# NVIDIA/OpenSeq2Seq

Hardware: AMD Instinct MI355X
Metric: audio-frames/sec/node Jasper10x5 bf16 (train step, objects = input feature frames) (higher is better)
Workload: dtype bf16; 1 GPU; Jasper 10x5 DR (jasper10x5_LibriSpeech_nvgrad_masks) full train step: log-mel front end from int16 PCM resident in HBM+fwd+bwd+NovoGrad/LARC/Backoff, B=32/GPU, durations U[2,16.7]s padded to the batch max, F=64, V=29; global_batch=32, parallelism=dp1, skipped_steps=0

## Files before the change

### openseq2seq_amd/csrc/conv1d_common.hpp

```cpp
#pragma once
#include <type_traits>

#include "os2s_common.hpp"

namespace os2s {

struct ConvArgs {
  const bf16_t* x;
  const bf16_t* w;
  void* y;
  const int32_t* in_len;
  const int32_t* out_len;
  const float* bias;
  float* stats;
  int B, Tin, Tout, Cin, Cout, K, stride, dil, padL;
  long long x_sb, x_st, y_sb, y_st;
  int out_f32, accumulate;
  int mtiles_per_b, MT, MT8, NT, nchunks, R, Rpad;
  int act;
  float keep_prob;
  unsigned long long seed;
  const bf16_t* residual;
  const bf16_t* mask_ref;
  float mask_scale;
  const bf16_t* stat_ref;
  float* ws_slabs;
  int* ws_cnt;
  int ws_nslabs, ncu;
  int force_split;
  unsigned long long* dbg;
  int dbg_fixed_w;
  int pp_tile = 0, pp_ok2 = 0, pp_ok3 = 0;
  float pp_c256 = 1.19f, pp_c2 = 0.90f, pp_c3 = 1.06f;
  int pp_prio = 0;
  float pp_dgrad_pen = 1.f;
  int tile_order = 0;
};

__device__ __forceinline__ void dma16(const void* gsrc, char* lds_wave_base) {
  __builtin_amdgcn_global_load_lds(
      (const __attribute__((address_space(1))) void*)gsrc,
      (__attribute__((address_space(3))) void*)lds_wave_base, 16, 0, 0);
}

constexpr size_t kEpiSplitBytes = 140 * 1024;
template <int BM, int BN, int NWIN, int NTHR>
constexpr size_t conv_epilogue_lds_bytes() {
  constexpr size_t OP = BN * 2 + 16;
  constexpr int EW = (NWIN * BM * OP > kEpiSplitBytes) ? 1 : NWIN;
  constexpr int RG = (NTHR / (BN / 2)) > 0 ? (NTHR / (BN / 2)) : 1;
  return (size_t)EW * BM * OP + (size_t)EW * RG * BN * 2 * 4;
}

constexpr int kMaxConvGroups = 16;
struct ConvGroup {
  const bf16_t* x;
  const bf16_t* w;
  void* y;
  float* stats;
  int Cin, Cout, accumulate, tile_begin;
  int x_st = 0, y_st = 0;
};
struct ConvGroupTable {
  int ngroups, total_tiles;
  ConvGroup g[kMaxConvGroups];
};
int launch_conv1x1_pp(hipStream_t stream, ConvArgs a, ConvGroupTable gt);

template <int BM, int BN, int WM, int WN, int NWIN>
__device__ __forceinline__ void conv_epilogue(const ConvArgs& p,
                                              f32x16 (&acc)[(BN / WN) / 32][((BM * NWIN) / WM) / 32],
                                              char* smem, int tid, int lane, int wid,
                                              const int (&wmid)[NWIN], int n0,
                                              const int (&wb)[NWIN], const int (&wt0)[NWIN]) {
  constexpr int NW = WM * WN, NTHR = NW * 64;
  constexpr int WTM = (BM * NWIN) / WM, WTN = BN / WN, MI = WTM / 32, NI = WTN / 32;
  const int wm = wid / WN, wn = wid % WN;
  constexpr bool STRADDLE = (BM % WTM) != 0;
  static_assert(!STRADDLE || (size_t)NWIN * BM * (BN * 2 + 16) <= kEpiSplitBytes,
                "a straddling wave layout needs all windows staged in one pass");
  const int my_win = (wm * WTM) / BM;
  const int row_in_win = (wm * WTM) % BM;
  const int my_b = (NWIN == 1 || my_win == 0) ? wb[0] : wb[NWIN - 1];
  const int my_t0 = (NWIN == 1 || my_win == 0) ? wt0[0] : wt0[NWIN - 1];
  const int my_mid = (NWIN == 1 || my_win == 0) ? wmid[0] : wmid[NWIN - 1];
  const int l31 = lane & 31, lhi = lane >> 5;
  if (p.out_f32) {
    const int b = my_b, t0 = my_t0;
    const int valid_rows = (my_mid >= 0) ? min(BM, p.Tout - t0) : 0;
    float* const yb = reinterpret_cast<float*>(p.y) + (long long)b * p.y_sb;
#pragma unroll
    for (int in = 0; in < NI; ++in)
#pragma unroll
      for (int im = 0; im < MI; ++im) {
        const int tt = row_in_win + im * 32 + l31;
#pragma unroll
        for (int e = 0; e < 16; ++e) {
          const int cc = n0 + wn * WTN + in * 32 + 8 * (e >> 2) + 4 * lhi + (e & 3);
          if (tt < valid_rows && cc < p.Cout) {
            float v = acc[in][im][e];
            if (p.bias) v += p.bias[cc];
            float* dst = yb + (long long)(t0 + tt) * p.y_st + cc;
            if (p.accumulate) v += *dst;
            *dst = v;
          }
        }
      }
    return;
  }

#ifdef OS2S_EPI_STAMPS
  unsigned long long* const est = (p.dbg && blockIdx.x < 2048) ? p.dbg + (size_t)blockIdx.x * 24 + 8 : nullptr;
  int esi = 0;
#define OS2S_EPI_STAMP() do { if (est && tid == 0 && esi < 16) est[esi] = __builtin_readcyclecounter(); ++esi; } while (0)
#else
#define OS2S_EPI_STAMP() do {} while (0)
#endif
  constexpr int OP = BN * 2 + 16;
  constexpr bool EPI_SPLIT = (size_t)NWIN * BM * OP > kEpiSplitBytes;
  constexpr int EW = EPI_SPLIT ? 1 : NWIN;
  char* const ot = smem;
#pragma unroll
  for (int w0 = 0; w0 < NWIN; w0 += EW) {
  OS2S_EPI_STAMP();
  __syncthreads();
  OS2S_EPI_STAMP();
  auto stage_tile = [&](auto DROP) {
  unsigned long long seed = p.seed;
  if constexpr (decltype(DROP)::value) asm volatile("" : "+s"(seed));
#pragma unroll
  for (int in = 0; in < NI; ++in)
#pragma unroll
    for (int im = 0; im < MI; ++im) {
      const int tt = wm * WTM + im * 32 + l31 - w0 * BM;
      const int b = my_b, t0 = my_t0 - (my_win - w0) * BM;
#pragma unroll
      for (int g = 0; g < 4; ++g) {
        const int cc = wn * WTN + in * 32 + 8 * g + 4 * lhi;
        float v0 = acc[in][im][4 * g + 0], v1 = acc[in][im][4 * g + 1];
        float v2 = acc[in][im][4 * g + 2], v3 = acc[in][im][4 * g + 3];
        if (p.bias) {
          const int gc = n0 + cc;
          if (gc + 3 < p.Cout) {
            v0 += p.bias[gc]; v1 += p.bias[gc + 1]; v2 += p.bias[gc + 2]; v3 += p.bias[gc + 3];
          }
        }
        if (p.act == 1) {
          v0 = fmaxf(v0, 0.f); v1 = fmaxf(v1, 0.f); v2 = fmaxf(v2, 0.f); v3 = fmaxf(v3, 0.f);
        } else if (p.act == 3) {
          v0 = fminf(fmaxf(v0, 0.f), 20.f); v1 = fminf(fmaxf(v1, 0.f), 20.f);
          v2 = fminf(fmaxf(v2, 0.f), 20.f); v3 = fminf(fmaxf(v3, 0.f), 20.f);
        }
        if constexpr (decltype(DROP)::value) {
          const long long e0 = ((long long)b * p.Tout + t0 + tt) * p.Cout + n0 + cc;
          const uint32_t bits = dropout_bits8(seed, (unsigned long long)(e0 >> 3), p.keep_prob) >>
                                (uint32_t)(e0 & 7);
          const float ik = 1.f / p.keep_prob;
          v0 = (bits & 1u) ? v0 * ik : 0.f;
          v1 = (bits & 2u) ? v1 * ik : 0.f;
          v2 = (bits & 4u) ? v2 * ik : 0.f;
          v3 = (bits & 8u) ? v3 * ik : 0.f;
        }
        u32x2 pk;
        pk[0] = pack2bf(v0, v1);
        pk[1] = pack2bf(v2, v3);
        *reinterpret_cast<u32x2*>(ot + tt * OP + cc * 2) = pk;
      }
    }
  };
  if constexpr (STRADDLE) {
    stage_tile(std::false_type{});
  } else if (my_win >= w0 && my_win < w0 + EW) {
    if (__builtin_amdgcn_readfirstlane(p.keep_prob < 1.f ? 1 : 0)) stage_tile(std::true_type{});
    else stage_tile(std::false_type{});
  }
  OS2S_EPI_STAMP();
  __syncthreads();
  OS2S_EPI_STAMP();

#pragma unroll
  for (int w = w0; w < w0 + EW; ++w) {
  const int b = wb[w], t0 = wt0[w];
  const int valid_rows = (wmid[w] >= 0) ? min(BM, p.Tout - t0) : 0;
  const char* const otw = ot + (w - w0) * BM * OP;
  bf16_t* const yb = reinterpret_cast<bf16_t*>(p.y) + (long long)b * p.y_sb;
  constexpr int NQ = (BM * (BN / 8) + NTHR - 1) / NTHR;
  static_assert((BM * (BN / 8)) % NTHR == 0, "whole number of chunks per thread");
  const bool inside = __builtin_amdgcn_readfirstlane((valid_rows == BM && n0 + BN <= p.Cout) ? 1 : 0);
  u32x4 v[NQ], ro[NQ], ao[NQ];
  if (inside) {
#pragma unroll
    for (int i = 0; i < NQ; ++i) {
      const int q = tid + i * NTHR;
      const int row = q / (BN / 8), c8 = q - row * (BN / 8);
      v[i] = *reinterpret_cast<const u32x4*>(otw + row * OP + c8 * 16);
      const long long off = (long long)(t0 + row) * p.y_st + n0 + c8 * 8;
      if (p.residual) ro[i] = *reinterpret_cast<const u32x4*>(p.residual + (long long)b * p.y_sb + off);
      if (p.accumulate) ao[i] = *reinterpret_cast<const u32x4*>(yb + off);
      if (p.mask_ref) ro[i] = *reinterpret_cast<const u32x4*>(p.mask_ref + (long long)b * p.y_sb + off);
    }
#pragma unroll
    for (int i = 0; i < NQ; ++i) {
      const int q = tid + i * NTHR;
      const int row = q / (BN / 8), c8 = q - row * (BN / 8);
      if (p.residual && !p.mask_ref) {
#pragma unroll
        for (int e = 0; e < 4; ++e)
          v[i][e] = pack2bf(bflo(v[i][e]) + bflo(ro[i][e]), bfhi(v[i][e]) + bfhi(ro[i][e]));
      }
      if (p.accumulate) {
#pragma unroll
        for (int e = 0; e < 4; ++e)
          v[i][e] = pack2bf(bflo(v[i][e]) + bflo(ao[i][e]), bfhi(v[i][e]) + bfhi(ao[i][e]));
      }
      if (p.mask_ref) {
#pragma unroll
        for (int e = 0; e < 4; ++e)
          v[i][e] = pack2bf(bflo(ro[i][e]) > 0.f ? bflo(v[i][e]) * p.mask_scale : 0.f,
                            bfhi(ro[i][e]) > 0.f ? bfhi(v[i][e]) * p.mask_scale : 0.f);
        if (p.stats) *reinterpret_cast<u32x4*>(const_cast<char*>(otw) + row * OP + c8 * 16) = v[i];
      }
      *reinterpret_cast<u32x4*>(yb + (long long)(t0 + row) * p.y_st + n0 + c8 * 8) = v[i];
    }
  } else {
    for (int i = 0; i < NQ; ++i) {
      const int q = tid + i * NTHR;
      const int row = q / (BN / 8), c8 = q - row * (BN / 8);
      const int gc = n0 + c8 * 8;
      if (row < valid_rows && gc < p.Cout) {
        u32x4 x = *reinterpret_cast<const u32x4*>(otw + row * OP + c8 * 16);
        bf16_t* dst = yb + (long long)(t0 + row) * p.y_st + gc;
        if (p.residual && !p.mask_ref) {
          const u32x4 o = *reinterpret_cast<const u32x4*>(
              p.residual + (long long)b * p.y_sb + (long long)(t0 + row) * p.y_st + gc);
#pragma unroll
          for (int e = 0; e < 4; ++e) x[e] = pack2bf(bflo(x[e]) + bflo(o[e]), bfhi(x[e]) + bfhi(o[e]));
        }
        if (p.accumulate) {
          const u32x4 o = *reinterpret_cast<const u32x4*>(dst);
#pragma unroll
          for (int e = 0; e < 4; ++e) x[e] = pack2bf(bflo(x[e]) + bflo(o[e]), bfhi(x[e]) + bfhi(o[e]));
        }
        if (p.mask_ref) {
          const u32x4 o = *reinterpret_cast<const u32x4*>(
              p.mask_ref + (long long)b * p.y_sb + (long long)(t0 + row) * p.y_st + gc);
#pragma unroll
          for (int e = 0; e < 4; ++e)
            x[e] = pack2bf(bflo(o[e]) > 0.f ? bflo(x[e]) * p.mask_scale : 0.f,
                           bfhi(o[e]) > 0.f ? bfhi(x[e]) * p.mask_scale : 0.f);
          if (p.stats) *reinterpret_cast<u32x4*>(const_cast<char*>(otw) + row * OP + c8 * 16) = x;
        }
        *reinterpret_cast<u32x4*>(dst) = x;
      }
    }
  }
  }

  OS2S_EPI_STAMP();
  if (p.stats && p.mask_ref) __syncthreads();
  if (p.stats) {
    constexpr int CP = BN / 2;
    constexpr int RG = (NTHR / CP) > 0 ? (NTHR / CP) : 1;
    constexpr int RPT = (BM + RG - 1) / RG;
    const int cp = tid % CP, rg = tid / CP;
#pragma unroll
    for (int w = w0; w < w0 + EW; ++w) {
      if (wmid[w] < 0) continue;
      const int valid_rows = min(BM, p.Tout - wt0[w]);
      const char* const otw = ot + (w - w0) * BM * OP;
      float s0 = 0.f, s1 = 0.f, q0 = 0.f, q1 = 0.f;
      if (rg < RG) {
        uint32_t vv[RPT];
#pragma unroll
        for (int i = 0; i < RPT; ++i) {
          const int row = rg + i * RG;
          vv[i] = row < valid_rows ? *reinterpret_cast<const uint32_t*>(otw + row * OP + cp * 4) : 0u;
        }
        if (p.stat_ref) {
          const bool cok = n0 + cp * 2 < p.Cout;
          const bf16_t* const rp = p.stat_ref + (long long)wb[w] * p.y_sb + (long long)wt0[w] * p.y_st + n0 + cp * 2;
          uint32_t rr[RPT];
#pragma unroll
          for (int i = 0; i < RPT; ++i) {
            const int row = rg + i * RG;
            rr[i] = (cok && row < valid_rows) ? *reinterpret_cast<const uint32_t*>(rp + (long long)row * p.y_st) : 0u;
          }
#pragma unroll
          for (int i = 0; i < RPT; ++i) {
            const float a = bflo(vv[i]), bb = bfhi(vv[i]);
            s0 += a; q0 += a * bflo(rr[i]);
            s1 += bb; q1 += bb * bfhi(rr[i]);
          }
        } else {
#pragma unroll
          for (int i = 0; i < RPT; ++i) {
            const float a = bflo(vv[i]), bb = bfhi(vv[i]);
            s0 += a; q0 += a * a;
            s1 += bb; q1 += bb * bb;
          }
        }
        float* sc = reinterpret_cast<float*>(smem + EW * BM * OP) + (size_t)(w - w0) * RG * BN * 2;
        sc[(rg * BN + cp * 2 + 0) * 2 + 0] = s0;
        sc[(rg * BN + cp * 2 + 0) * 2 + 1] = q0;
        sc[(rg * BN + cp * 2 + 1) * 2 + 0] = s1;
        sc[(rg * BN + cp * 2 + 1) * 2 + 1] = q1;
      }
    }
    OS2S_EPI_STAMP();
    __syncthreads();
    OS2S_EPI_STAMP();
#pragma unroll
    for (int w = w0; w < w0 + EW; ++w) {
      if (wmid[w] < 0) continue;
      const float* sc = reinterpret_cast<const float*>(smem + EW * BM * OP) + (size_t)(w - w0) * RG * BN * 2;
      for (int c = tid; c < BN; c += NTHR) {
        float s = 0.f, qq = 0.f;
#pragma unroll
        for (int g = 0; g < RG; ++g) {
          s += sc[(g * BN + c) * 2 + 0];
          qq += sc[(g * BN + c) * 2 + 1];
        }
        const int gc = n0 + c;
        if (gc < p.Cout) {
          p.stats[((long long)wmid[w] * 2 + 0) * p.Cout + gc] = s;
          p.stats[((long long)wmid[w] * 2 + 1) * p.Cout + gc] = qq;
        }
      }
    }
  }
  }
}

}
```

Baseline: 967,800 frames/sec.

## Fuse stats reduction into conv epilogue store pass with buffer loads and prefetch

Rewrites the conv epilogue's write-out phase so the per-channel sum/sumsq statistics are computed in the same pass that applies residual/accumulate/mask and stores the output. The separate stats pass that reread the staged tile from LDS, and the barrier before it, go away. Global reads and writes now use raw buffer loads and stores with range-clamped resources, which replaces the explicit boundary branches. The next batch's residual/accumulate/mask loads are issued before the current batch is stored, to overlap memory latency. When stats are enabled it switches to 8-byte pieces and processes two windows per half-block. This risks higher register pressure and subtle correctness issues in the reduction layout and out-of-range handling.

```diff
diff --git a/openseq2seq_amd/csrc/conv1d_common.hpp b/openseq2seq_amd/csrc/conv1d_common.hpp
--- a/openseq2seq_amd/csrc/conv1d_common.hpp
+++ b/openseq2seq_amd/csrc/conv1d_common.hpp
@@ -67,6 +67,14 @@
 };
 int launch_conv1x1_pp(hipStream_t stream, ConvArgs a, ConvGroupTable gt);
 
+__device__ __forceinline__ __amdgpu_buffer_rsrc_t epi_rsrc(const void* base, long long elem_off, int bytes) {
+  const unsigned long long a = (unsigned long long)base + (unsigned long long)elem_off * 2ull;
+  const unsigned lo = __builtin_amdgcn_readfirstlane((unsigned)a);
+  const unsigned hi = __builtin_amdgcn_readfirstlane((unsigned)(a >> 32));
+  return __builtin_amdgcn_make_buffer_rsrc((void*)(((unsigned long long)hi << 32) | lo), 0,
+                                           __builtin_amdgcn_readfirstlane(bytes), 0x00020000);
+}
+
 template <int BM, int BN, int WM, int WN, int NWIN>
 __device__ __forceinline__ void conv_epilogue(const ConvArgs& p,
                                               f32x16 (&acc)[(BN / WN) / 32][((BM * NWIN) / WM) / 32],
@@ -119,7 +127,10 @@
   constexpr int OP = BN * 2 + 16;
   constexpr bool EPI_SPLIT = (size_t)NWIN * BM * OP > kEpiSplitBytes;
   constexpr int EW = EPI_SPLIT ? 1 : NWIN;
+  constexpr int CP = BN / 2;
+  constexpr int RG = (NTHR / CP) > 0 ? (NTHR / CP) : 1;
   char* const ot = smem;
+
 #pragma unroll
   for (int w0 = 0; w0 < NWIN; w0 += EW) {
   OS2S_EPI_STAMP();
@@ -174,138 +185,163 @@
     if (__builtin_amdgcn_readfirstlane(p.keep_prob < 1.f ? 1 : 0)) stage_tile(std::true_type{});
     else stage_tile(std::false_type{});
   }
+  auto run_windows = [&](auto W16) {
+  constexpr bool WIDE = decltype(W16)::value;
+  constexpr int PB = WIDE ? 16 : 8, PD = PB / 4;
+  using piece_t = std::conditional_t<WIDE, u32x4, u32x2>;
+  constexpr int LR = BN * 2 / PB;
+  constexpr int TPW = WIDE ? NTHR : NTHR / 2;
+  constexpr int RGM = TPW / LR;
+  constexpr int RPT = BM / RGM;
+  static_assert(BM % RGM == 0 && TPW % 64 == 0 && (WIDE || RGM == RG), "whole waves per window; the chains of the sums");
+  constexpr int NROUND = WIDE ? EW : (EW + 1) / 2;
+  constexpr int NQB = WIDE ? ((NW > 4 || RPT % 2) ? RPT : RPT / 2) : ((NW > 4 && RPT % 16 == 0) ? 16 : 8);
+  static_assert(RPT % NQB == 0, "whole batches per window");
+  constexpr int NBT = RPT / NQB;
+  const int half = WIDE ? 0 : __builtin_amdgcn_readfirstlane(tid / TPW);
+  const int th = tid - half * TPW, c4 = th % LR, rg = th / LR;
+  const int y_st2 = (int)p.y_st * 2;
+  const int voff0 = (n0 + c4 * (PB / 2) < p.Cout) ? rg * y_st2 + (n0 + c4 * (PB / 2)) * 2 : (int)0x80000000;
+  const int vstep = RGM * y_st2;
+  auto ld = [&](__amdgpu_buffer_rsrc_t rs, int off) -> piece_t {
+    if constexpr (WIDE) return __builtin_amdgcn_raw_buffer_load_b128(rs, off, 0, 0);
+    else return __builtin_amdgcn_raw_buffer_load_b64(rs, off, 0, 0);
+  };
+
+  piece_t ro[NQB], ao[NQB], sr[NQB];
+  int mb = 0, mt0 = 0, mmid = -1, mslot = 0;
+  auto my_rows = [&]() { return (mmid >= 0) ? max(0, min(BM, p.Tout - mt0)) : 0; };
+  auto my_rsrc = [&](const void* base) {
+    const int rows = my_rows();
+    return epi_rsrc(base, (long long)mb * p.y_sb + (long long)mt0 * p.y_st,
+                    (base && rows > 0) ? ((rows - 1) * (int)p.y_st + p.Cout) * 2 : 0);
+  };
+  auto issue_loads = [&](int i0) {
+    if (p.mask_ref || p.residual) {
+      const __amdgpu_buffer_rsrc_t rs = my_rsrc(p.mask_ref ? p.mask_ref : p.residual);
+#pragma unroll
+      for (int i = 0; i < NQB; ++i) ro[i] = ld(rs, voff0 + (i0 + i) * vstep);
+    }
+    if (p.accumulate) {
+      const __amdgpu_buffer_rsrc_t rs = my_rsrc(p.y);
+#pragma unroll
+      for (int i = 0; i < NQB; ++i) ao[i] = ld(rs, voff0 + (i0 + i) * vstep);
+    }
+    if constexpr (!WIDE) {
+      if (p.stat_ref) {
+        const __amdgpu_buffer_rsrc_t rs = my_rsrc(p.stat_ref);
+#pragma unroll
+        for (int i = 0; i < NQB; ++i) sr[i] = ld(rs, voff0 + (i0 + i) * vstep);
+      }
+    }
+  };
+  auto pick_window = [&](int r) {
+    if constexpr (WIDE) {
+      mb = wb[w0 + r]; mt0 = wt0[w0 + r]; mmid = wmid[w0 + r]; mslot = r;
+    } else {
+      const int wa = w0 + 2 * r, wb1 = wa + 1 < w0 + EW ? wa + 1 : wa;
+      const bool second = wa + 1 < w0 + EW;
+      mb = half ? wb[wb1] : wb[wa];
+      mt0 = half ? wt0[wb1] : wt0[wa];
+      mmid = half ? (second ? wmid[wb1] : -1) : wmid[wa];
+      mslot = second ? 2 * r + half : 2 * r;
+    }
+  };
+
+  pick_window(0);
+  issue_loads(0);
   OS2S_EPI_STAMP();
   __syncthreads();
   OS2S_EPI_STAMP();
 
-#pragma unroll
-  for (int w = w0; w < w0 + EW; ++w) {
-  const int b = wb[w], t0 = wt0[w];
-  const int valid_rows = (wmid[w] >= 0) ? min(BM, p.Tout - t0) : 0;
-  const char* const otw = ot + (w - w0) * BM * OP;
-  bf16_t* const yb = reinterpret_cast<bf16_t*>(p.y) + (long long)b * p.y_sb;
-  constexpr int NQ = (BM * (BN / 8) + NTHR - 1) / NTHR;
-  static_assert((BM * (BN / 8)) % NTHR == 0, "whole number of chunks per thread");
-  const bool inside = __builtin_amdgcn_readfirstlane((valid_rows == BM && n0 + BN <= p.Cout) ? 1 : 0);
-  u32x4 v[NQ], ro[NQ], ao[NQ];
-  if (inside) {
-#pragma unroll
-    for (int i = 0; i < NQ; ++i) {
-      const int q = tid + i * NTHR;
-      const int row = q / (BN / 8), c8 = q - row * (BN / 8);
-      v[i] = *reinterpret_cast<const u32x4*>(otw + row * OP + c8 * 16);
-      const long long off = (long long)(t0 + row) * p.y_st + n0 + c8 * 8;
-      if (p.residual) ro[i] = *reinterpret_cast<const u32x4*>(p.residual + (long long)b * p.y_sb + off);
-      if (p.accumulate) ao[i] = *reinterpret_cast<const u32x4*>(yb + off);
-      if (p.mask_ref) ro[i] = *reinterpret_cast<const u32x4*>(p.mask_ref + (long long)b * p.y_sb + off);
-    }
-#pragma unroll
-    for (int i = 0; i < NQ; ++i) {
-      const int q = tid + i * NTHR;
-      const int row = q / (BN / 8), c8 = q - row * (BN / 8);
+  float s[4], q[4];
+#pragma unroll
+  for (int u = 0; u < NROUND * NBT; ++u) {
+    const int i0 = (u % NBT) * NQB;
+    const int valid_rows = my_rows();
+    const char* const otw = ot + mslot * BM * OP;
+    piece_t v[NQB];
+#pragma unroll
+    for (int i = 0; i < NQB; ++i)
+      v[i] = *reinterpret_cast<const piece_t*>(otw + (rg + (i0 + i) * RGM) * OP + c4 * PB);
+    if (i0 == 0) {
+#pragma unroll
+      for (int e = 0; e < 4; ++e) s[e] = q[e] = 0.f;
+    }
+#pragma unroll
+    for (int i = 0; i < NQB; ++i) {
+      if constexpr (!WIDE) {
+        if (!p.mask_ref) {
+          const bool live = rg + (i0 + i) * RGM < valid_rows;
+#pragma unroll
+          for (int e = 0; e < PD; ++e) {
+            const uint32_t x = live ? v[i][e] : 0u;
+            const float a = bflo(x), bb = bfhi(x);
+            s[2 * e] += a; q[2 * e] += a * a;
+            s[2 * e + 1] += bb; q[2 * e + 1] += bb * bb;
+          }
+        }
+      }
       if (p.residual && !p.mask_ref) {
 #pragma unroll
-        for (int e = 0; e < 4; ++e)
+        for (int e = 0; e < PD; ++e)
           v[i][e] = pack2bf(bflo(v[i][e]) + bflo(ro[i][e]), bfhi(v[i][e]) + bfhi(ro[i][e]));
       }
       if (p.accumulate) {
 #pragma unroll
-        for (int e = 0; e < 4; ++e)
+        for (int e = 0; e < PD; ++e)
           v[i][e] = pack2bf(bflo(v[i][e]) + bflo(ao[i][e]), bfhi(v[i][e]) + bfhi(ao[i][e]));
       }
       if (p.mask_ref) {
 #pragma unroll
-        for (int e = 0; e < 4; ++e)
+        for (int e = 0; e < PD; ++e)
           v[i][e] = pack2bf(bflo(ro[i][e]) > 0.f ? bflo(v[i][e]) * p.mask_scale : 0.f,
                             bfhi(ro[i][e]) > 0.f ? bfhi(v[i][e]) * p.mask_scale : 0.f);
-        if (p.stats) *reinterpret_cast<u32x4*>(const_cast<char*>(otw) + row * OP + c8 * 16) = v[i];
-      }
-      *reinterpret_cast<u32x4*>(yb + (long long)(t0 + row) * p.y_st + n0 + c8 * 8) = v[i];
-    }
-  } else {
-    for (int i = 0; i < NQ; ++i) {
-      const int q = tid + i * NTHR;
-      const int row = q / (BN / 8), c8 = q - row * (BN / 8);
-      const int gc = n0 + c8 * 8;
-      if (row < valid_rows && gc < p.Cout) {
-        u32x4 x = *reinterpret_cast<const u32x4*>(otw + row * OP + c8 * 16);
-        bf16_t* dst = yb + (long long)(t0 + row) * p.y_st + gc;
-        if (p.residual && !p.mask_ref) {
-          const u32x4 o = *reinterpret_cast<const u32x4*>(
-              p.residual + (long long)b * p.y_sb + (long long)(t0 + row) * p.y_st + gc);
-#pragma unroll
-          for (int e = 0; e < 4; ++e) x[e] = pack2bf(bflo(x[e]) + bflo(o[e]), bfhi(x[e]) + bfhi(o[e]));
-        }
-        if (p.accumulate) {
-          const u32x4 o = *reinterpret_cast<const u32x4*>(dst);
-#pragma unroll
-          for (int e = 0; e < 4; ++e) x[e] = pack2bf(bflo(x[e]) + bflo(o[e]), bfhi(x[e]) + bfhi(o[e]));
-        }
-        if (p.mask_ref) {
-          const u32x4 o = *reinterpret_cast<const u32x4*>(
-              p.mask_ref + (long long)b * p.y_sb + (long long)(t0 + row) * p.y_st + gc);
-#pragma unroll
-          for (int e = 0; e < 4; ++e)
-            x[e] = pack2bf(bflo(o[e]) > 0.f ? bflo(x[e]) * p.mask_scale : 0.f,
-                           bfhi(o[e]) > 0.f ? bfhi(x[e]) * p.mask_scale : 0.f);
-          if (p.stats) *reinterpret_cast<u32x4*>(const_cast<char*>(otw) + row * OP + c8 * 16) = x;
-        }
-        *reinterpret_cast<u32x4*>(dst) = x;
-      }
-    }
-  }
-  }
-
-  OS2S_EPI_STAMP();
-  if (p.stats && p.mask_ref) __syncthreads();
+        if constexpr (!WIDE) {
+          if (p.stat_ref) {
+#pragma unroll
+            for (int e = 0; e < PD; ++e) {
+              const float a = bflo(v[i][e]), bb = bfhi(v[i][e]);
+              s[2 * e] += a; q[2 * e] += a * bflo(sr[i][e]);
+              s[2 * e + 1] += bb; q[2 * e + 1] += bb * bfhi(sr[i][e]);
+            }
+          } else {
+#pragma unroll
+            for (int e = 0; e < PD; ++e) {
+              const float a = bflo(v[i][e]), bb = bfhi(v[i][e]);
+              s[2 * e] += a; q[2 * e] += a * a;
+              s[2 * e + 1] += bb; q[2 * e + 1] += bb * bb;
+            }
+          }
+        }
+      }
+      __builtin_amdgcn_sched_barrier(0);
+    }
+    const __amdgpu_buffer_rsrc_t yrs = my_rsrc(p.y);
+    const int voff_st = voff0 + i0 * vstep;
+    if constexpr (!WIDE) {
+      if (i0 + NQB == RPT && mmid >= 0) {
+        float* sc = reinterpret_cast<float*>(smem + EW * BM * OP) + (size_t)mslot * RG * BN * 2 + (rg * BN + c4 * 4) * 2;
+#pragma unroll
+        for (int e = 0; e < 4; ++e) { sc[2 * e] = s[e]; sc[2 * e + 1] = q[e]; }
+      }
+    }
+    if (u + 1 < NROUND * NBT) {
+      if ((u + 1) % NBT == 0) pick_window((u + 1) / NBT);
+      issue_loads(((u + 1) % NBT) * NQB);
+    }
+#pragma unroll
+    for (int i = 0; i < NQB; ++i) {
+      if constexpr (WIDE) __builtin_amdgcn_raw_buffer_store_b128(v[i], yrs, voff_st + i * vstep, 0, 0);
+      else __builtin_amdgcn_raw_buffer_store_b64(v[i], yrs, voff_st + i * vstep, 0, 0);
+    }
+  }
+  };
+  if (p.stats) run_windows(std::false_type{});
+  else run_windows(std::true_type{});
+
+  OS2S_EPI_STAMP();
   if (p.stats) {
-    constexpr int CP = BN / 2;
-    constexpr int RG = (NTHR / CP) > 0 ? (NTHR / CP) : 1;
-    constexpr int RPT = (BM + RG - 1) / RG;
-    const int cp = tid % CP, rg = tid / CP;
-#pragma unroll
-    for (int w = w0; w < w0 + EW; ++w) {
-      if (wmid[w] < 0) continue;
-      const int valid_rows = min(BM, p.Tout - wt0[w]);
-      const char* const otw = ot + (w - w0) * BM * OP;
-      float s0 = 0.f, s1 = 0.f, q0 = 0.f, q1 = 0.f;
-      if (rg < RG) {
-        uint32_t vv[RPT];
-#pragma unroll
-        for (int i = 0; i < RPT; ++i) {
-          const int row = rg + i * RG;
-          vv[i] = row < valid_rows ? *reinterpret_cast<const uint32_t*>(otw + row * OP + cp * 4) : 0u;
-        }
-        if (p.stat_ref) {
-          const bool cok = n0 + cp * 2 < p.Cout;
-          const bf16_t* const rp = p.stat_ref + (long long)wb[w] * p.y_sb + (long long)wt0[w] * p.y_st + n0 + cp * 2;
-          uint32_t rr[RPT];
-#pragma unroll
-          for (int i = 0; i < RPT; ++i) {
-            const int row = rg + i * RG;
-            rr[i] = (cok && row < valid_rows) ? *reinterpret_cast<const uint32_t*>(rp + (long long)row * p.y_st) : 0u;
-          }
-#pragma unroll
-          for (int i = 0; i < RPT; ++i) {
-            const float a = bflo(vv[i]), bb = bfhi(vv[i]);
-            s0 += a; q0 += a * bflo(rr[i]);
-            s1 += bb; q1 += bb * bfhi(rr[i]);
-          }
-        } else {
-#pragma unroll
-          for (int i = 0; i < RPT; ++i) {
-            const float a = bflo(vv[i]), bb = bfhi(vv[i]);
-            s0 += a; q0 += a * a;
-            s1 += bb; q1 += bb * bb;
-          }
-        }
-        float* sc = reinterpret_cast<float*>(smem + EW * BM * OP) + (size_t)(w - w0) * RG * BN * 2;
-        sc[(rg * BN + cp * 2 + 0) * 2 + 0] = s0;
-        sc[(rg * BN + cp * 2 + 0) * 2 + 1] = q0;
-        sc[(rg * BN + cp * 2 + 1) * 2 + 0] = s1;
-        sc[(rg * BN + cp * 2 + 1) * 2 + 1] = q1;
-      }
-    }
     OS2S_EPI_STAMP();
     __syncthreads();
     OS2S_EPI_STAMP();
@@ -327,8 +363,9 @@
         }
       }
     }
-  }
-  }
-}
-
-}
+    OS2S_EPI_STAMP();
+  }
+  }
+}
+
+}
```

Measured after the change: 973,600 frames/sec, median of 6. Within noise of the previous version (+0.6%).
